# MarwanNour/SEAL-FYP-Logistic-Regression

Measured on AMD Instinct MI355X. Metric: CKKS ciphertext rotate+plain-mult ops/sec at N=16384; HBM GB/s vs roofline, higher is better.
Workload: dtype u64; 1 GPU; C3: N=16384, coeff_modulus bits [60, 40, 40, 40, 40, 60], level L=5 (k=6); per step and per GPU 4608 independent rotate_vector(step=1, direct Galois key)+multiply_plain, uniform random residues drawn on the device, inputs resident in HBM; batch_per_gpu=4608, parallelism=1 x independent ciphertext batches (no data-path collective), algorithmic_bytes_per_op=11141120

## Files before the change

### seal_fyp_logistic_regression_amd/csrc/hefx_keyswitch.hip

```cpp
#include <cstdio>
#include <cstdlib>
#include "hefx_internal.h"
#include "hefx_ntt.cuh"
#include "hefx_ntt8.cuh"

template <int LOGN>
struct KsWaves {
#ifdef HEFX_WAVES
    static constexpr int INV = HEFX_WAVES, FWD = HEFX_WAVES;
#else
    static constexpr int INV = LOGN <= 14 ? 2 : 4;
    static constexpr int FWD = LOGN <= 13 ? 2 : 4;
#endif
    static constexpr int NB_INV = (INV <= 2 && LOGN <= 13) ? 1 : 2, NB_FWD = (FWD <= 2 && LOGN < 13) ? 1 : 2;
};

namespace hefx {

typedef u64 u64x2_t __attribute__((ext_vector_type(2)));
__device__ __forceinline__ ulonglong2 nt_load16(const u64 *p)
{
    const u64x2_t v = __builtin_nontemporal_load(reinterpret_cast<const u64x2_t *>(p));
    return make_ulonglong2(v.x, v.y);
}
// ... 209 lines not shown
    struct Ctx {
        ModConst mc;
    };
    __device__ static __forceinline__ Ctx make(const ModConst &mc, const ModConstF &) { return Ctx{mc}; }
    typedef ulonglong2 X;
    struct K {
        ulonglong2 k0, k1;
    };
    __device__ static __forceinline__ X xin(const ulonglong2 &bits, bool, const Ctx &) { return bits; }
    __device__ static __forceinline__ K kin(const ulonglong2 &k0, const ulonglong2 &k1, const Ctx &) { return K{k0, k1}; }
    u64 a0xl = 0, a0xh = 0, a0yl = 0, a0yh = 0, a1xl = 0, a1xh = 0, a1yl = 0, a1yh = 0;
    __device__ __forceinline__ void mac(const X &x, const K &k, const Ctx &)
    {
        mac128(a0xl, a0xh, x.x, k.k0.x);
        mac128(a0yl, a0yh, x.y, k.k0.y);
        mac128(a1xl, a1xh, x.x, k.k1.x);
        mac128(a1yl, a1yh, x.y, k.k1.y);
    }
    __device__ __forceinline__ void mac_diag(const MacW &in, const ulonglong2 &dg, const Ctx &c)
    {
        ulonglong2 r0, r1;
        in.result(r0, r1, c);
        mac128(a0xl, a0xh, r0.x, dg.x);
        mac128(a0yl, a0yh, r0.y, dg.y);
        mac128(a1xl, a1xh, r1.x, dg.x);
        mac128(a1yl, a1yh, r1.y, dg.y);
    }
    template <bool LT2Q = false>
    __device__ __forceinline__ void result_data(ulonglong2 &r0, ulonglong2 &r1, const Ctx &c) const { result<LT2Q>(r0, r1, c); }
    template <bool LT2Q = false>
    __device__ __forceinline__ void result(ulonglong2 &r0, ulonglong2 &r1, const Ctx &c) const
    {
        r0.x = LT2Q ? barrett128_lt2q(a0xl, a0xh, c.mc) : barrett128(a0xl, a0xh, c.mc);
        r0.y = LT2Q ? barrett128_lt2q(a0yl, a0yh, c.mc) : barrett128(a0yl, a0yh, c.mc);
        r1.x = LT2Q ? barrett128_lt2q(a1xl, a1xh, c.mc) : barrett128(a1xl, a1xh, c.mc);
        r1.y = LT2Q ? barrett128_lt2q(a1yl, a1yh, c.mc) : barrett128(a1yl, a1yh, c.mc);
    }
};

struct MacL {
    typedef MacW::Ctx Ctx;
    __device__ static __forceinline__ Ctx make(const ModConst &mc, const ModConstF &) { return Ctx{mc}; }
    struct X {
        uint32_t xl, xh, yl, yh;
    };
    struct K {
        uint32_t k0xl, k0xh, k0yl, k0yh, k1xl, k1xh, k1yl, k1yh;
    };
    __device__ static __forceinline__ uint32_t lo30(u64 v) { return (uint32_t)v & 0x3FFFFFFFu; }
    __device__ static __forceinline__ uint32_t hi30(u64 v) { return (uint32_t)(v >> 30); }
    __device__ static __forceinline__ X xin(const ulonglong2 &b, bool, const Ctx &)
    {
        return X{lo30(b.x), hi30(b.x), lo30(b.y), hi30(b.y)};
    }
    __device__ static __forceinline__ K kin(const ulonglong2 &k0, const ulonglong2 &k1, const Ctx &)
    {
        return K{lo30(k0.x), hi30(k0.x), lo30(k0.y), hi30(k0.y), lo30(k1.x), hi30(k1.x), lo30(k1.y), hi30(k1.y)};
    }
    u64 c[4][3] = {};
    __device__ static __forceinline__ void mad(u64 (&col)[3], uint32_t xl, uint32_t xh, uint32_t kl, uint32_t kh)
    {
        col[0] += (u64)xl * kl;
        col[1] += (u64)xl * kh;
        col[1] += (u64)xh * kl;
        col[2] += (u64)xh * kh;
    }
    __device__ __forceinline__ void mac(const X &x, const K &k, const Ctx &)
    {
        mad(c[0], x.xl, x.xh, k.k0xl, k.k0xh);
        mad(c[1], x.yl, x.yh, k.k0yl, k.k0yh);
        mad(c[2], x.xl, x.xh, k.k1xl, k.k1xh);
        mad(c[3], x.yl, x.yh, k.k1yl, k.k1yh);
    }
    __device__ __forceinline__ void mac_diag(const MacL &in, const ulonglong2 &dg, const Ctx &cx)
    {
        ulonglong2 r0, r1;
        in.result(r0, r1, cx);
        const uint32_t dxl = lo30(dg.x), dxh = hi30(dg.x), dyl = lo30(dg.y), dyh = hi30(dg.y);
        mad(c[0], lo30(r0.x), hi30(r0.x), dxl, dxh);
        mad(c[1], lo30(r0.y), hi30(r0.y), dyl, dyh);
        mad(c[2], lo30(r1.x), hi30(r1.x), dxl, dxh);
        mad(c[3], lo30(r1.y), hi30(r1.y), dyl, dyh);
    }
    template <bool LT2Q>
    __device__ static __forceinline__ u64 fold(const u64 (&col)[3], const ModConst &mc)
    {
        u64 lo = col[0], hi = 0, t = col[1] << 30;
        lo += t;
        hi += (col[1] >> 34) + (lo < t);
        t = col[2] << 60;
        lo += t;
        hi += (col[2] >> 4) + (lo < t);
        return LT2Q ? barrett128_lt2q(lo, hi, mc) : barrett128(lo, hi, mc);
    }
    template <bool LT2Q = false>
    __device__ __forceinline__ void result_data(ulonglong2 &r0, ulonglong2 &r1, const Ctx &cx) const { result<LT2Q>(r0, r1, cx); }
    template <bool LT2Q = false>
    __device__ __forceinline__ void result(ulonglong2 &r0, ulonglong2 &r1, const Ctx &cx) const
    {
        r0.x = fold<LT2Q>(c[0], cx.mc);
        r0.y = fold<LT2Q>(c[1], cx.mc);
        r1.x = fold<LT2Q>(c[2], cx.mc);
        r1.y = fold<LT2Q>(c[3], cx.mc);
    }
};

struct MacF {
    typedef ArithF64::Ctx Ctx;
    __device__ static __forceinline__ Ctx make(const ModConst &, const ModConstF &mf) { return ArithF64::make(mf); }
    typedef double2 X;
    struct K {
        double k0x, k0y, k1x, k1y;
    };
    __device__ static __forceinline__ X xin(const ulonglong2 &b, bool own, const Ctx &)
    {
        return own ? make_double2(ArithF64::from_u64(b.x), ArithF64::from_u64(b.y))
                   : make_double2(__longlong_as_double((long long)b.x), __longlong_as_double((long long)b.y));
    }
    __device__ static __forceinline__ K kin(const ulonglong2 &k0, const ulonglong2 &k1, const Ctx &)
    {
        return K{ArithF64::from_u64(k0.x), ArithF64::from_u64(k0.y), ArithF64::from_u64(k1.x), ArithF64::from_u64(k1.y)};
    }
    double a0x = 0.0, a0y = 0.0, a1x = 0.0, a1y = 0.0;
    __device__ __forceinline__ void mac(const X &x, const K &k, const Ctx &c)
    {
        a0x += ArithF64::mm(x.x, k.k0x, c);
        a0y += ArithF64::mm(x.y, k.k0y, c);
        a1x += ArithF64::mm(x.x, k.k1x, c);
        a1y += ArithF64::mm(x.y, k.k1y, c);
    }
    __device__ __forceinline__ void mac_diag(const MacF &in, const ulonglong2 &dg, const Ctx &c)
    {
        const double dx = ArithF64::from_u64(dg.x), dy = ArithF64::from_u64(dg.y);
        a0x += ArithF64::mm(in.a0x, dx, c);
        a0y += ArithF64::mm(in.a0y, dy, c);
        a1x += ArithF64::mm(in.a1x, dx, c);
        a1y += ArithF64::mm(in.a1y, dy, c);
    }
    template <bool LT2Q = false>
    __device__ __forceinline__ void result_data(ulonglong2 &r0, ulonglong2 &r1, const Ctx &) const
    {
        r0.x = ArithF64::raw(a0x), r0.y = ArithF64::raw(a0y), r1.x = ArithF64::raw(a1x), r1.y = ArithF64::raw(a1y);
    }
    template <bool LT2Q = false>
    __device__ __forceinline__ void result(ulonglong2 &r0, ulonglong2 &r1, const Ctx &c) const
    {
        r0.x = ArithF64::canon(a0x, c);
        r0.y = ArithF64::canon(a0y, c);
        r1.x = ArithF64::canon(a1x, c);
        r1.y = ArithF64::canon(a1y, c);
    }
};

__device__ __forceinline__ bool slot_is_f64(const DevTables &T, int L, int jj)
{
    return T.modsf[jj < L ? jj : T.k - 1].q != 0.0;
}
__device__ __forceinline__ int nth_int_slot(const DevTables &T, int L, int y)
{
    int jj = 0;
    for (;; ++jj) {
        if (slot_is_f64(T, L, jj)) continue;
        if (y == 0) break;
        --y;
    }
    return jj;
}

template <class F>
__device__ __forceinline__ void mac_dispatch(const DevTables &T, int m, int L, const F &f)
{
    if (T.modsf[m].q != 0.0)
        f(MacF());
    else if (L <= 8 && (T.mods[m].q >> 60) == 0)
        f(MacL());
    else
        f(MacW());
}

template <bool STREAM>
__device__ __forceinline__ void mac_store(u64 *acc0, u64 *acc1, size_t w, const ulonglong2 &r0, const ulonglong2 &r1)
{
    if (STREAM) {
        nt_store16(acc0 + 2 * w, r0.x, r0.y);
        nt_store16(acc1 + 2 * w, r1.x, r1.y);
    } else {
        gst16(acc0 + 2 * w, r0);
        gst16(acc1 + 2 * w, r1);
    }
}

template <class P, int NI, bool STREAM, class XR>
__device__ __forceinline__ void mac_items(const DevTables &T, const u64 *key, int L, int jj, int m, size_t n, size_t w,
                                          const u64 *const (&own)[NI], const uint32_t (&own_elt)[NI], const XR &xrow,
                                          u64 *const (&acc0)[NI], u64 *const (&acc1)[NI])
{
    const typename P::Ctx cx = P::make(T.mods[m], T.modsf[m]);
    const int logn = T.logn;
    const size_t kpoly = (size_t)T.k * n;
    P A[NI];
    auto load_k = [&](int i, ulonglong2 &k0, ulonglong2 &k1) {
        const u64 *kb = key + ((size_t)i * 2 * T.k + m) * n;
        k0 = gld16(kb + 2 * w);
        k1 = gld16(kb + kpoly + 2 * w);
    };
    auto load_x = [&](int i, ulonglong2 (&xb)[NI]) {
#pragma unroll
        for (int e = 0; e < NI; ++e) {
            const u64 *xp = xrow(e, i) + 2 * w;
            xb[e] = STREAM ? nt_load16(xp) : gld16(xp);
        }
    };
    if (jj < L) {
        ulonglong2 xb[NI], k0, k1;
#pragma unroll
        for (int e = 0; e < NI; ++e) xb[e] = gather_pair(own[e], (uint32_t)w, own_elt[e], logn);
        load_k(jj, k0, k1);
        const typename P::K k = P::kin(k0, k1, cx);
#pragma unroll
        for (int e = 0; e < NI; ++e) A[e].mac(P::xin(xb[e], true, cx), k, cx);
    }
    constexpr int G = 1;
    auto digit_at = [&](int r) { return r < jj ? r : r + 1; };
    const int nd = jj < L ? L - 1 : L;
    int r0 = 0;
    for (; r0 + G <= nd; r0 += G) {
        ulonglong2 xb[G][NI], k0[G], k1[G];
#pragma unroll
        for (int g = 0; g < G; ++g) {
            load_x(digit_at(r0 + g), xb[g]);
            load_k(digit_at(r0 + g), k0[g], k1[g]);
        }
        HEFX_STAGE_FENCE();
#pragma unroll
        for (int g = 0; g < G; ++g) {
            const typename P::K k = P::kin(k0[g], k1[g], cx);
#pragma unroll
            for (int e = 0; e < NI; ++e) A[e].mac(P::xin(xb[g][e], false, cx), k, cx);
        }
    }
    for (; r0 < nd; ++r0) {
        ulonglong2 xb[NI], k0, k1;
        load_x(digit_at(r0), xb);
        load_k(digit_at(r0), k0, k1);
        const typename P::K k = P::kin(k0, k1, cx);
#pragma unroll
        for (int e = 0; e < NI; ++e) A[e].mac(P::xin(xb[e], false, cx), k, cx);
    }
#pragma unroll
    for (int e = 0; e < NI; ++e) {
        ulonglong2 r0, r1;
        if (jj < L) {
#ifdef HEFX_NO_LT2Q
            A[e].result_data(r0, r1, cx);
#else
            A[e].template result_data<true>(r0, r1, cx);
#endif
        } else {
#ifdef HEFX_NO_LT2Q
            A[e].result(r0, r1, cx);
#else
            A[e].template result<true>(r0, r1, cx);
#endif
        }
        mac_store<STREAM>(acc0[e], acc1[e], w, r0, r1);
    }
}

template <bool STREAM>
__device__ __forceinline__ void mac_unit(const DevTables &T, const KsItem *__restrict__ items, int L, int relin, int item0,
                                         int count, const KsScratch &S, int jj, int bl0, size_t w)
{
    const size_t n = (size_t)1 << T.logn;
    const int m = jj < L ? jj : T.k - 1;
    const bool two = bl0 + 1 < count;
    const KsItem it0 = items[item0 + bl0], it1 = items[item0 + bl0 + (two ? 1 : 0)];
    const int ownrow = jj < L ? jj : 0;
    const u64 *const own[2] = {it0.c_in + ((size_t)(relin ? 2 * L : L) + ownrow) * n,
                               it1.c_in + ((size_t)(relin ? 2 * L : L) + ownrow) * n};
    const uint32_t own_elt[2] = {relin ? 1u : item_elt(it0), relin ? 1u : item_elt(it1)};
    auto xrow2 = [&](int e, int i) { return S.x + (((size_t)(bl0 + e) * L + i) * (L + 1) + jj) * n; };
    auto accrow = [&](int bl, int c) { return S.acc + (((size_t)(item0 + bl) * 2 + c) * (L + 1) + jj) * n; };
    u64 *const acc0[2] = {accrow(bl0, 0), accrow(bl0 + 1, 0)}, *const acc1[2] = {accrow(bl0, 1), accrow(bl0 + 1, 1)};
    mac_dispatch(T, m, L, [&](auto pol) {
        using P = decltype(pol);
        if (two && it1.key == it0.key) {
            mac_items<P, 2, STREAM>(T, it0.key, L, jj, m, n, w, own, own_elt, xrow2, acc0, acc1);
        } else {
            const u64 *const o0[1] = {own[0]}, *const o1[1] = {own[1]};
            const uint32_t e0[1] = {own_elt[0]}, e1[1] = {own_elt[1]};
            u64 *const a00[1] = {acc0[0]}, *const a01[1] = {acc1[0]}, *const a10[1] = {acc0[1]}, *const a11[1] = {acc1[1]};
            mac_items<P, 1, STREAM>(T, it0.key, L, jj, m, n, w, o0, e0, [&](int, int i) { return xrow2(0, i); }, a00, a01);
            if (two)
                mac_items<P, 1, STREAM>(T, it1.key, L, jj, m, n, w, o1, e1, [&](int, int i) { return xrow2(1, i); }, a10, a11);
        }
    });
}

template <bool STREAM>
__global__ __launch_bounds__(256) void ks_mac_kernel(DevTables T, const KsItem *__restrict__ items, int L, int relin,
                                                     int item0, int count, int int_only, KsScratch S)
{
    if (S.gate_mode == 2 && ks_gated_out(S)) return;
    const int jj = int_only ? nth_int_slot(T, L, blockIdx.y) : (int)blockIdx.y;
#ifdef HEFX_STAMP
    const int wg = blockIdx.x + gridDim.x * (blockIdx.y + gridDim.y * blockIdx.z);
    if (threadIdx.x == 0 && wg < 1024) hefx_stamp_buf[((size_t)2 * 1024 + wg) * 16] = wall_clock64();
#endif
    mac_unit<STREAM>(T, items, L, relin, item0, count, S, jj, 2 * blockIdx.z, (size_t)blockIdx.x * blockDim.x + threadIdx.x);
#ifdef HEFX_STAMP
    if (HEFX_STAMP > 1) asm volatile("s_waitcnt vmcnt(0) lgkmcnt(0)" ::: "memory");
    if (threadIdx.x == 0 && wg < 1024) hefx_stamp_buf[((size_t)2 * 1024 + wg) * 16 + 15] = wall_clock64();
#endif
}

template <int LOGN>
__global__ __launch_bounds__(SplitCfg<LOGN>::T, KsWaves<LOGN>::FWD) void ks_ntt_digits_kernel(DevTables T, int L, int rows,
                                                                             int item0, int stream_x, KsScratch S)
{
    extern __shared__ __align__(16) u64 lds[];
    HEFX_STAMP_KERNEL(1);
    HEFX_STAMP_AT(0);
    ntt_digit_row<LOGN>(T, L, rows, item0, stream_x, S, lds);
    HEFX_STAMP_AT(15);
}

template <class P>
__device__ __forceinline__ void mac_gathered(P &A, const typename P::Ctx &cx, const DevTables &T, const KsItem &it,
                                             const u64 *__restrict__ c1, const KsScratch &S, int L, int jj, int m,
                                             size_t n, size_t w)
{
    const uint2 pi = gld_u32x2(it.perm + 2 * w);
    for (int i = 0; i < L; ++i) {
        const u64 *__restrict__ xrow = i == jj ? c1 + (size_t)i * n : S.x + ((size_t)i * (L + 1) + jj) * n;
        ulonglong2 xb;
        xb.x = gld8(xrow + pi.x);
        xb.y = gld8(xrow + pi.y);
        const u64 *kbase = it.key + ((size_t)i * 2 * T.k + m) * n;
        const ulonglong2 k0 = gld16(kbase + 2 * w);
        const ulonglong2 k1 = gld16(kbase + (size_t)T.k * n + 2 * w);
        A.mac(P::xin(xb, i == jj, cx), P::kin(k0, k1, cx), cx);
    }
}

__global__ __launch_bounds__(256) void ks_mac_exact_kernel(DevTables T, const KsItem *__restrict__ items, int L, KsScratch S)
{
    const size_t n = (size_t)1 << T.logn;
    const int jj = blockIdx.y, b = blockIdx.z;
    const int m = jj < L ? jj : T.k - 1;
    const size_t w = (size_t)blockIdx.x * blockDim.x + threadIdx.x;
    const KsItem it = items[b];
    if (w == 0 && jj == 0 && b == 0 && *S.gate == S.gate_tag) atomicAdd(S.gate_hits, 1u);
    const u64 *__restrict__ c1 = it.c_in + (size_t)L * n;
    const u64 *__restrict__ xs = S.x + (size_t)it.dsrc * L * (L + 1) * n;
    mac_dispatch(T, m, L, [&](auto pol) {
        using P = decltype(pol);
        const typename P::Ctx cx = P::make(T.mods[m], T.modsf[m]);
        P A, B;
        const uint32_t p0 = gld_u32x2(it.perm + 2 * w).x;
        const ulonglong2 wv = gld16(it.flipw + (size_t)m * n + 2 * w);
        auto load = [&](int i, const u64 *__restrict__ xrow, ulonglong2 &xb, ulonglong2 &k0, ulonglong2 &k1) {
            xb = gld16(xrow + (p0 & ~1u));
            const u64 *kbase = it.key + ((size_t)i * 2 * T.k + m) * n;
            k0 = gld16(kbase + 2 * w);
            k1 = gld16(kbase + (size_t)T.k * n + 2 * w);
        };
        auto swapped = [&](const ulonglong2 &v) { return (p0 & 1u) ? make_ulonglong2(v.y, v.x) : v; };
        if (jj < L) {
            ulonglong2 xb, k0, k1;
            load(jj, c1 + (size_t)jj * n, xb, k0, k1);
            A.mac(P::xin(swapped(xb), true, cx), P::kin(k0, k1, cx), cx);
        }
        constexpr int G = 1;
        auto digit_at = [&](int r) { return r < jj ? r : r + 1; };
        auto term = [&](int i, const ulonglong2 &xb, const ulonglong2 &k0, const ulonglong2 &k1) {
            const typename P::K k = P::kin(k0, k1, cx);
            A.mac(P::xin(swapped(xb), false, cx), k, cx);
            const u64 c = S.qmod[(size_t)i * T.k + m];
            B.mac(P::xin(make_ulonglong2(c, c), true, cx), k, cx);
        };
        const int nd = jj < L ? L - 1 : L;
        int r = 0;
        for (; r + G <= nd; r += G) {
            ulonglong2 xb[G], k0[G], k1[G];
#pragma unroll
            for (int g = 0; g < G; ++g) {
                const int i = digit_at(r + g);
                load(i, xs + ((size_t)i * (L + 1) + jj) * n, xb[g], k0[g], k1[g]);
            }
            HEFX_STAGE_FENCE();
#pragma unroll
            for (int g = 0; g < G; ++g) term(digit_at(r + g), xb[g], k0[g], k1[g]);
        }
        for (; r < nd; ++r) {
            const int i = digit_at(r);
            ulonglong2 xb, k0, k1;
            load(i, xs + ((size_t)i * (L + 1) + jj) * n, xb, k0, k1);
            term(i, xb, k0, k1);
        }
        ulonglong2 r0, r1, f0, f1;
        P C;
        C.mac_diag(B, wv, cx);
        if constexpr (std::is_same<P, MacF>::value) {
            if (jj < L) {
                P S2 = A;
                S2.a0x += C.a0x, S2.a0y += C.a0y, S2.a1x += C.a1x, S2.a1y += C.a1y;
                S2.result_data(r0, r1, cx);
            } else {
                A.result(r0, r1, cx);
                C.result(f0, f1, cx);
                const u64 q = T.mods[m].q;
                r0.x = addmod(r0.x, f0.x, q), r0.y = addmod(r0.y, f0.y, q);
                r1.x = addmod(r1.x, f1.x, q), r1.y = addmod(r1.y, f1.y, q);
            }
        } else {
            A.result(r0, r1, cx);
            C.result(f0, f1, cx);
            const u64 q = T.mods[m].q;
            r0.x = addmod(r0.x, f0.x, q);
            r0.y = addmod(r0.y, f0.y, q);
            r1.x = addmod(r1.x, f1.x, q);
            r1.y = addmod(r1.y, f1.y, q);
        }
        mac_store<false>(S.acc + (((size_t)b * 2 + 0) * (L + 1) + jj) * n, S.acc + (((size_t)b * 2 + 1) * (L + 1) + jj) * n,
                         w, r0, r1);
    });
}

__global__ __launch_bounds__(256) void flip_mask_kernel(DevTables T, const uint32_t *__restrict__ ginv, u64 *__restrict__ rows)
{
    const uint32_t n = 1u << T.logn;
    const uint32_t c = blockIdx.x * blockDim.x + threadIdx.x;
    const uint32_t e = blockIdx.z, m = blockIdx.y;
    rows[((size_t)e * T.k + m) * n + c] = ((c * ginv[e]) & (2 * n - 1)) >> T.logn;
}

constexpr int LT2_CHUNK = 8;

__global__ __launch_bounds__(256) void lt2_mac_kernel(DevTables T, const KsItem *__restrict__ items, int L, int nrot,
                                                      KsScratch S, const u64 *__restrict__ src_c1 ,
                                                      u64 *__restrict__ partial )
{
    const size_t n = (size_t)1 << T.logn;
    const int jj = blockIdx.y, ch = blockIdx.z;
    const int m = jj < L ? jj : T.k - 1;
    const size_t w = (size_t)blockIdx.x * blockDim.x + threadIdx.x;
    const int l0 = ch * LT2_CHUNK, l1 = l0 + LT2_CHUNK < nrot ? l0 + LT2_CHUNK : nrot;
    mac_dispatch(T, m, L, [&](auto pol) {
        using P = decltype(pol);
        const typename P::Ctx cx = P::make(T.mods[m], T.modsf[m]);
        P tot;
        for (int l = l0; l < l1; ++l) {
            const KsItem it = items[l];
            P A;
            mac_gathered(A, cx, T, it, src_c1, S, L, jj, m, n, w);
            tot.mac_diag(A, gld16(it.pt + (size_t)m * n + 2 * w), cx);
        }
        ulonglong2 r0, r1;
        tot.result(r0, r1, cx);
        u64 *base = partial + (size_t)ch * 2 * (L + 1) * n;
        mac_store<false>(base + (size_t)jj * n, base + ((size_t)(L + 1) + jj) * n, w, r0, r1);
    });
}

__global__ __launch_bounds__(256) void lt2_c0_kernel(DevTables T, const KsItem *__restrict__ items, int L, int nrot,
                                                     const u64 *__restrict__ c0, u64 *__restrict__ partial )
{
    const size_t n = (size_t)1 << T.logn;
    const int j = blockIdx.y, ch = blockIdx.z;
    const ModConst mc = T.mods[j];
    const size_t w = (size_t)blockIdx.x * blockDim.x + threadIdx.x;
    u64 xl = 0, xh = 0, yl = 0, yh = 0;
    const int l0 = ch * LT2_CHUNK, l1 = l0 + LT2_CHUNK < nrot ? l0 + LT2_CHUNK : nrot;
    const u64 *__restrict__ row = c0 + (size_t)j * n;
    for (int l = l0; l < l1; ++l) {
        const KsItem it = items[l];
        const uint2 pi = gld_u32x2(it.perm + 2 * w);
// ... 743 lines not shown
    int slot, g;
    fan_decode(4 * L, g, slot);
    const int j = slot >> 2, part = slot & 3;
    if (g >= rows) return;
    const int t = threadIdx.x;
    const int sp = T.k - 1;
    const ModConst mcp = T.mods[sp];
    const ModConstF mfp = T.modsf[sp];
    const NttTables ntp = ntt_tables(T, sp);
    const u64 *__restrict__ plane = S.u + (size_t)g * QC::N + (size_t)part * QC::Q;
    u64 v[8];
    if (mfp.q != 0.0)
        quarter_inv_planes<LOGN, ArithF64>(v, plane, lds, ntp.itwf, ArithF64::make(mfp), t);
    else
        quarter_inv_planes<LOGN, ArithU64>(v, plane, lds, ntp.itw, ArithU64::make(mcp), t);
    HEFX_STAMP_AT(15);
    HEFX_STAMP_KERNEL(4);
    HEFX_STAMP_AT(0);
    const u64 half = mcp.q >> 1;
#pragma unroll
    for (int r = 0; r < 8; ++r) v[r] = csub(v[r] + half, mcp.q);
    const ModConst mc = T.mods[j];
    const ModConstF mf = T.modsf[j];
    const InMode mode = {true, true, true, T.halfmod[(size_t)sp * T.k + j], true, mcp.q < 2 * mc.q};
    u64 *__restrict__ fd = S.x + ((size_t)g * L + j) * QC::N + (size_t)part * QC::Q;
    const NttTables nt = ntt_tables(T, j);
    fwd_policy_dispatch(mc, mf, [&](auto pol) {
        using A = decltype(pol);
        const typename A::Ctx cx = make_ctx(A{}, mc, mf);
        typename A::V f[8];
        fwd_inputs8<A>(f, v, mode, cx, mc);
        ntt8_fwd_core<LOGN - 2, A>(f, reinterpret_cast<typename A::V *>(lds), fwd_tw(A{}, nt), cx, t, 1);
#pragma unroll
        for (int r = 0; r < 8; r += 2) gst16(fd + C::idx_out(t, r), make_ulonglong2(A::raw(f[r]), A::raw(f[r + 1])));
    });
    HEFX_STAMP_AT(15);
}

template <int LOGN, class A>
__device__ __forceinline__ void pair_finish_body(const DevTables &T, const KsItem &it, int L, int relin, int b, int c, int j,
                                                 uint32_t g, const KsScratch &S)
{
    constexpr size_t N = (size_t)1 << LOGN, Q = N / 4;
    const int sp = T.k - 1;
    const ModConst mc = T.mods[j];
    const ModConstF mf = T.modsf[j];
    const typename A::Ctx cx = make_ctx(A{}, mc, mf);
    const auto pinv = md_pinv(A{}, T, sp, j);
    const typename A::TW *__restrict__ tw = fwd_tw(A{}, ntt_tables(T, j));
    const typename A::TW wb = tw[Q + g], wa0 = tw[2 * Q + 2 * g], wa1 = tw[2 * Q + 2 * g + 1];
    const u64 *__restrict__ fp = S.x + (((size_t)b * 2 + c) * L + j) * N + g;
    typename A::V p0 = A::unraw(gld8(fp)), p1 = A::unraw(gld8(fp + Q)), p2 = A::unraw(gld8(fp + 2 * Q)),
                  p3 = A::unraw(gld8(fp + 3 * Q));
    const size_t w4 = 4 * (size_t)g;
    const u64 *__restrict__ acc = S.acc + (((size_t)b * 2 + c) * (L + 1) + j) * N + w4;
    const ulonglong2 a01 = gld16(acc), a23 = gld16(acc + 2);
    const u64 *__restrict__ addrow = it.c_in + ((size_t)(relin ? c : 0) * L + j) * N;
    const bool has_add = relin || c == 0;
    const uint32_t elt = relin ? 1u : item_elt(it);
    const u64 *__restrict__ pt = it.pt ? it.pt + (size_t)j * N + w4 : nullptr;
    u64 *__restrict__ dst = it.c_out + ((size_t)c * L + j) * N + w4;
    auto epilogue = [&](auto has_add_c, auto has_pt_c) {
        constexpr bool HA = decltype(has_add_c)::value, HP = decltype(has_pt_c)::value;
        ulonglong2 s01 = make_ulonglong2(0, 0), s23 = s01, t01 = s01, t23 = s01;
        if constexpr (HA) {
            s01 = gather_pair(addrow, 2 * g, elt, LOGN);
            s23 = gather_pair(addrow, 2 * g + 1, elt, LOGN);
        }
        if constexpr (HP) {
            t01 = gld16(pt);
            t23 = gld16(pt + 2);
        }
        fwd_last_two<LOGN, A>(p0, p1, p2, p3, wb, wa0, wa1, cx);
        ulonglong2 o01, o23;
        o01.x = md_epilogue(A{}, p0, a01.x, s01.x, t01.x, HP, cx, pinv, mc);
        o01.y = md_epilogue(A{}, p1, a01.y, s01.y, t01.y, HP, cx, pinv, mc);
        o23.x = md_epilogue(A{}, p2, a23.x, s23.x, t23.x, HP, cx, pinv, mc);
        o23.y = md_epilogue(A{}, p3, a23.y, s23.y, t23.y, HP, cx, pinv, mc);
        gst16(dst, o01);
        gst16(dst + 2, o23);
        if constexpr (!HP) {
            if (it.acc_out) {
                const size_t arow = ((size_t)c * L + j) * N + w4;
                const ulonglong2 i01 = gld16(it.acc_in + arow), i23 = gld16(it.acc_in + arow + 2);
                gst16(it.acc_out + arow, make_ulonglong2(addmod(i01.x, o01.x, mc.q), addmod(i01.y, o01.y, mc.q)));
                gst16(it.acc_out + arow + 2, make_ulonglong2(addmod(i23.x, o23.x, mc.q), addmod(i23.y, o23.y, mc.q)));
            }
        }
    };
    if (has_add) {
        if (pt)
            epilogue(std::true_type{}, std::true_type{});
        else
            epilogue(std::true_type{}, std::false_type{});
    } else {
        if (pt)
            epilogue(std::false_type{}, std::true_type{});
        else
            epilogue(std::false_type{}, std::false_type{});
    }
}

template <int LOGN>
__global__ __launch_bounds__(256) void ks_pair_finish_kernel(DevTables T, const KsItem *__restrict__ items, int L, int relin,
                                                            KsScratch S)
{
    const int row = blockIdx.y, b = blockIdx.z;
    const int c = row / L, j = row % L;
    const uint32_t g = blockIdx.x * blockDim.x + threadIdx.x;
#ifdef HEFX_STAMP
    const int wg = blockIdx.x + gridDim.x * (blockIdx.y + gridDim.y * blockIdx.z);
    if (threadIdx.x == 0 && wg < 1024) hefx_stamp_buf[((size_t)5 * 1024 + wg) * 16] = wall_clock64();
#endif
    const KsItem it = items[b];
    const ModConst mc = T.mods[j];
    fwd_policy_dispatch(mc, T.modsf[j], [&](auto pol) {
        using A = decltype(pol);
        pair_finish_body<LOGN, A>(T, it, L, relin, b, c, j, g, S);
    });
#ifdef HEFX_STAMP
    if (HEFX_STAMP > 1) asm volatile("s_waitcnt vmcnt(0) lgkmcnt(0)" ::: "memory");
    if (threadIdx.x == 0 && wg < 1024) hefx_stamp_buf[((size_t)5 * 1024 + wg) * 16 + 15] = wall_clock64();
#endif
}

template <typename K>
static void set_lds(K kernel, size_t bytes)
{
    (void)hipFuncSetAttribute(reinterpret_cast<const void *>(kernel), hipFuncAttributeMaxDynamicSharedMemorySize,
                              (int)bytes);
}

template <int LOGN>
static hipError_t launch_keyswitch_chunk_t(const DevTables &T, int L, int n, const KsItem *batch, bool relin,
                                           const KsScratch &scr, int sub, bool alias,
                                           const KsSmallItems *small, int quarter, hipStream_t s, KsProf *prof, int nsrc)
{
    using SC = SplitCfg<LOGN>;
    const size_t lds = SC::LDS_BYTES;
    auto lds_knob = [lds](const char *name) {
        const char *e = getenv(name);
        const size_t v = e ? (size_t)atol(e) : 0;
        return v > lds ? v : lds;
    };
    static const size_t lds_fin = lds_knob("HEFX_FIN_LDS"), lds_ntt = lds_knob("HEFX_NTT_LDS"),
                        lds_intt = lds_knob("HEFX_INTT_LDS"), lds_mdi = lds_knob("HEFX_MDI_LDS");
    static PerDeviceOnce attr_once;
    if (attr_once.first()) {
        set_lds(ks_intt_digits_kernel<LOGN>, lds_intt);
        set_lds(ks_intt_digits_small_kernel<LOGN>, lds);
        set_lds(ks_ntt_digits_kernel<LOGN>, lds_ntt);
        set_lds(ks_moddown_intt_kernel<LOGN>, lds_mdi);
        set_lds(ks_moddown_finish_kernel<LOGN>, lds_fin);
        if (getenv("HEFX_DEBUG")) {
            int nb = -1;
            (void)hipOccupancyMaxActiveBlocksPerMultiprocessor(&nb, ks_ntt_digits_kernel<LOGN>, SC::T, lds);
            fprintf(stderr, "[hefx] ks_ntt_digits_kernel<%d>: %d threads, %zu B LDS -> %d workgroups/CU\n", LOGN, SC::T,
                    lds, nb);
        }
    }
    const int rl = relin ? 1 : 0;
    auto mark = [&](int stage) {
        if (prof && prof->used < prof->cap) {
            (void)hipEventRecord(prof->ev[prof->used], s);
            prof->stage[prof->used++] = stage;
        }
    };
    if (nsrc > 0) {
        KsScratch hs = scr, fb = scr;
        hs.gate_mode = 1;
        fb.gate_mode = 2;
        mark(1);
        hipLaunchKernelGGL((ks_intt_digits_kernel<LOGN>), dim3(split_grid(nsrc * L)), dim3(SC::T), lds_intt, s, T, batch + n, L,
                           0, 1, nsrc * L, hs);
        mark(2);
        hipLaunchKernelGGL((ks_ntt_digits_kernel<LOGN>), dim3(group_grid(nsrc * L, L)), dim3(SC::T), lds_ntt, s, T, L, nsrc * L,
                           0, 0, hs);
        mark(3);
        hipLaunchKernelGGL(ks_mac_exact_kernel, dim3(SC::N / 2 / 256, L + 1, n), dim3(256), 0, s, T, batch, L, hs);
        mark(4);
        hipLaunchKernelGGL((ks_moddown_intt_kernel<LOGN>), dim3(split_grid(n * 2)), dim3(SC::T), lds_mdi, s, T, L, n * 2, hs);
        mark(5);
        hipLaunchKernelGGL((ks_moddown_finish_kernel<LOGN>), dim3(group_grid(n * 2, L)), dim3(SC::T), lds_fin, s, T, batch, L,
                           0, n * 2, hs);
        mark(7);
        hipLaunchKernelGGL((ks_intt_digits_kernel<LOGN>), dim3(split_grid(n * L)), dim3(SC::T), lds_intt, s, T, batch, L, 0, 0,
                           n * L, fb);
        hipLaunchKernelGGL((ks_ntt_digits_kernel<LOGN>), dim3(group_grid(n * L, L)), dim3(SC::T), lds_ntt, s, T, L, n * L, 0, 0,
                           fb);
        hipLaunchKernelGGL(ks_mac_kernel<false>, dim3(SC::N / 2 / 256, L + 1, (n + 1) / 2), dim3(256), 0, s, T, batch, L, 0, 0, n,
                           0, fb);
        hipLaunchKernelGGL((ks_moddown_intt_kernel<LOGN>), dim3(split_grid(n * 2)), dim3(SC::T), lds_mdi, s, T, L, n * 2, fb);
        hipLaunchKernelGGL((ks_moddown_finish_kernel<LOGN>), dim3(group_grid(n * 2, L)), dim3(SC::T), lds_fin, s, T, batch, L,
                           0, n * 2, fb);
        mark(-1);
        return hipGetLastError();
    }
    if (small && (quarter & KS_Q_PAIR) && sub >= n) {
        static PerDeviceOnce attrp;
        const size_t ldsq = QuarterCfg<LOGN>::LDS_BYTES;
        if (attrp.first()) {
            set_lds(ks_pair_digits_kernel<LOGN>, ldsq);
            set_lds(ks_pair_moddown_kernel<LOGN>, ldsq);
        }
        constexpr int TQ = QuarterCfg<LOGN>::T;
        mark(1);
        hipLaunchKernelGGL((ks_pair_digits_kernel<LOGN>), fan_grid(n * L, 4 * L), dim3(TQ), ldsq, s, T, *small,
                           const_cast<KsItem *>(batch), n, L, rl, n * L, scr);
        mark(3);
        hipLaunchKernelGGL((ks_pair_mac_kernel<LOGN>), dim3(SC::N / 4 / 256, 2 * (L + 1), n), dim3(256), 0, s, T, batch, L, rl,
                           scr);
        mark(4);
        hipLaunchKernelGGL((ks_pair_moddown_kernel<LOGN>), fan_grid(n * 2, 4 * L), dim3(TQ), ldsq, s, T, L, n * 2,
                           scr);
        mark(5);
        hipLaunchKernelGGL((ks_pair_finish_kernel<LOGN>), dim3(SC::N / 4 / 256, 2 * L, n), dim3(256), 0, s, T, batch, L, rl,
                           scr);
        mark(-1);
        return hipGetLastError();
    }
    static const bool heavy_on = !(getenv("HEFX_HEAVY_FIRST") && atoi(getenv("HEFX_HEAVY_FIRST")) == 0);
    static const int heavy_max = getenv("HEFX_HEAVY_MAX") ? atoi(getenv("HEFX_HEAVY_MAX")) : 640;
    auto heavy_order = [&](int m) { return heavy_on && m * L * L * 2 <= heavy_max ? 2 : 0; };
    if (small && (quarter & KS_Q_ALL) && sub >= n) {
        static PerDeviceOnce attrq;
        const size_t ldsq = QuarterCfg<LOGN>::LDS_BYTES;
        if (attrq.first()) {
            set_lds(ks_intt_digits_q_kernel<LOGN>, ldsq);
            set_lds(ks_ntt_digits_q_kernel<LOGN>, ldsq);
            set_lds(ks_moddown_intt_q_kernel<LOGN>, ldsq);
            set_lds(ks_moddown_finish_q_kernel<LOGN>, ldsq);
        }
        constexpr int TQ = QuarterCfg<LOGN>::T;
        mark(1);
        if (quarter & KS_Q_INTT)
            hipLaunchKernelGGL((ks_intt_digits_q_kernel<LOGN>), dim3(quarter_grid(n * L)), dim3(TQ), ldsq, s, T, *small,
                               const_cast<KsItem *>(batch), n, L, rl, n * L, scr);
        else
            hipLaunchKernelGGL((ks_intt_digits_small_kernel<LOGN>), dim3(split_grid(n * L)), dim3(SC::T), lds, s, T, *small,
                               const_cast<KsItem *>(batch), n, L, rl, n * L, scr);
        mark(2);
        if (quarter & KS_Q_NTT)
            hipLaunchKernelGGL((ks_ntt_digits_q_kernel<LOGN>), fan_grid(n * L, 4 * L), dim3(TQ), ldsq, s, T, L,
                               n * L, scr);
        else
            hipLaunchKernelGGL((ks_ntt_digits_kernel<LOGN>), dim3(group_grid(n * L, L)), dim3(SC::T), lds_ntt, s, T, L,
                               n * L, 0, heavy_order(n), scr);
        mark(3);
        hipLaunchKernelGGL(ks_mac_kernel<false>, dim3(SC::N / 2 / 256, L + 1, (n + 1) / 2), dim3(256), 0, s, T, batch, L, rl, 0,
                           n, 0, scr);
        mark(4);
        if (quarter & KS_Q_MDI)
            hipLaunchKernelGGL((ks_moddown_intt_q_kernel<LOGN>), dim3(quarter_grid(n * 2)), dim3(TQ), ldsq, s, T, L, n * 2,
                               scr);
        else
            hipLaunchKernelGGL((ks_moddown_intt_kernel<LOGN>), dim3(split_grid(n * 2)), dim3(SC::T), lds_mdi, s, T, L, n * 2,
                               scr);
        mark(5);
        if (quarter & KS_Q_FIN)
            hipLaunchKernelGGL((ks_moddown_finish_q_kernel<LOGN>), fan_grid(n * 2, 4 * L), dim3(TQ), ldsq, s, T,
                               batch, L, rl, n * 2, scr);
        else
            hipLaunchKernelGGL((ks_moddown_finish_kernel<LOGN>), dim3(group_grid(n * 2, L)), dim3(SC::T), lds_fin, s, T,
                               batch, L, rl, n * 2, scr);
        mark(-1);
        return hipGetLastError();
    }
    static const int force_stream_x = getenv("HEFX_STREAM_X") ? atoi(getenv("HEFX_STREAM_X")) : -1;
    auto stream_x_of = [&](int m) {
        return force_stream_x >= 0 ? force_stream_x : ((size_t)m * L * (L + 1) * SC::N * 8 > ((size_t)256 << 20) ? 1 : 0);
    };
    if (alias) {
        mark(0);
        hipLaunchKernelGGL(ks_alias_copy_kernel, dim3(SC::N / 2 / 256, 2 * L, n), dim3(256), 0, s, T, batch, L);
    }
    mark(1);
    if (small)
        hipLaunchKernelGGL((ks_intt_digits_small_kernel<LOGN>), dim3(split_grid(n * L)), dim3(SC::T), lds, s, T, *small,
                           const_cast<KsItem *>(batch), n, L, rl, n * L, scr);
    else
        hipLaunchKernelGGL((ks_intt_digits_kernel<LOGN>), dim3(split_grid(n * L)), dim3(SC::T), lds_intt, s, T, batch, L, rl, 0,
                           n * L, scr);
    if (sub < 0) {
        if constexpr (LOGN <= 14) {
            static PerDeviceOnce fattr;
            if (fattr.first()) set_lds(ks_ntt_macf_kernel<LOGN>, FusedCfg<LOGN>::LDS_BYTES);
            const int code = -sub - 1, nf = code & 0xff;
            const bool special_int = (code >> 8) & 1;
            const int nint = L + 1 - nf;
            const int pairs = special_int ? (nint - 1) * (L - 1) + L : nint * (L - 1);
            const int per_item = 2 * (nf + pairs);
            const int stream_x = (size_t)n * pairs * SC::N * 8 > ((size_t)256 << 20) ? 1 : 0;
            mark(6);
            hipLaunchKernelGGL((ks_ntt_macf_kernel<LOGN>), dim3(((n + 7) / 8) * 8 * per_item), dim3(FusedCfg<LOGN>::T),
                               FusedCfg<LOGN>::LDS_BYTES, s, T, batch, L, rl, n, nf, per_item, stream_x, scr);
            if (nint > 0) {
                mark(3);
                if (stream_x)
                    hipLaunchKernelGGL(ks_mac_kernel<true>, dim3(SC::N / 2 / 256, nint, (n + 1) / 2), dim3(256), 0, s, T, batch,
                                       L, rl, 0, n, 1, scr);
                else
                    hipLaunchKernelGGL(ks_mac_kernel<false>, dim3(SC::N / 2 / 256, nint, (n + 1) / 2), dim3(256), 0, s, T, batch,
                                       L, rl, 0, n, 1, scr);
            }
        }
    } else
    for (int item0 = 0; item0 < n; item0 += sub) {
        const int m = n - item0 < sub ? n - item0 : sub;
        mark(2);
        const int stream_x = stream_x_of(m);
        hipLaunchKernelGGL((ks_ntt_digits_kernel<LOGN>), dim3(group_grid(m * L, L)), dim3(SC::T), lds_ntt, s, T, L, m * L,
                           item0, stream_x | heavy_order(m), scr);
        mark(3);
        if (stream_x)
            hipLaunchKernelGGL(ks_mac_kernel<true>, dim3(SC::N / 2 / 256, L + 1, (m + 1) / 2), dim3(256), 0, s, T, batch,
                               L, rl, item0, m, 0, scr);
        else
            hipLaunchKernelGGL(ks_mac_kernel<false>, dim3(SC::N / 2 / 256, L + 1, (m + 1) / 2), dim3(256), 0, s, T, batch,
                               L, rl, item0, m, 0, scr);
    }
    mark(4);
    hipLaunchKernelGGL((ks_moddown_intt_kernel<LOGN>), dim3(split_grid(n * 2)), dim3(SC::T), lds_mdi, s, T, L, n * 2, scr);
    mark(5);
    hipLaunchKernelGGL((ks_moddown_finish_kernel<LOGN>), dim3(group_grid(n * 2, L)), dim3(SC::T), lds_fin, s, T, batch, L,
                       rl, n * 2, scr);
    mark(-1);
    return hipGetLastError();
}

__global__ __launch_bounds__(256) void lt2_reduce_kernel(DevTables T, int L, int period, int rows, int chunks,
                                                         const u64 *__restrict__ partial, const u64 *addin, u64 *out)
{
    const size_t n = (size_t)1 << T.logn;
    const int r = blockIdx.y;
    const int jj = r % period;
    const u64 q = T.mods[jj < L ? jj : T.k - 1].q;
    const size_t w = (size_t)blockIdx.x * blockDim.x + threadIdx.x;
    ulonglong2 acc = addin ? reinterpret_cast<const ulonglong2 *>(addin + (size_t)r * n)[w] : make_ulonglong2(0, 0);
    for (int ch = 0; ch < chunks; ++ch) {
        const ulonglong2 v = reinterpret_cast<const ulonglong2 *>(partial + ((size_t)ch * rows + r) * n)[w];
        acc.x = addmod(acc.x, v.x, q);
        acc.y = addmod(acc.y, v.y, q);
    }
    if (period == L + 1 && jj < L && T.modsf[jj].q != 0.0)
        acc = make_ulonglong2(ArithF64::raw(ArithF64::from_u64(acc.x)), ArithF64::raw(ArithF64::from_u64(acc.y)));
    reinterpret_cast<ulonglong2 *>(out + (size_t)r * n)[w] = acc;
}

template <int LOGN>
static hipError_t launch_lt2_decompose_t(const DevTables &T, int L, const KsItem *src_item, const KsItem *rot_items,
                                         int nrot, const KsScratch &scr, const u64 *ct_new, u64 *partial_s,
                                         u64 *partial_c0, u64 *cbuf, hipStream_t s)
{
    using SC = SplitCfg<LOGN>;
    const size_t lds = SC::LDS_BYTES;
    static PerDeviceOnce attr_once;
    if (attr_once.first()) {
        set_lds(ks_intt_digits_kernel<LOGN>, lds);
        set_lds(ks_ntt_digits_kernel<LOGN>, lds);
        set_lds(ks_moddown_intt_kernel<LOGN>, lds);
        set_lds(ks_moddown_finish_kernel<LOGN>, lds);
    }
    const int chunks = (nrot + LT2_CHUNK - 1) / LT2_CHUNK;
    hipLaunchKernelGGL((ks_intt_digits_kernel<LOGN>), dim3(split_grid(L)), dim3(SC::T), lds, s, T, src_item, L, 0, 1, L,
                       scr);
    hipLaunchKernelGGL((ks_ntt_digits_kernel<LOGN>), dim3(group_grid(L, L)), dim3(SC::T), lds, s, T, L, L, 0, 0, scr);
    hipLaunchKernelGGL(lt2_mac_kernel, dim3(SC::N / 2 / 256, L + 1, chunks), dim3(256), 0, s, T, rot_items, L, nrot, scr,
                       ct_new + (size_t)L * SC::N, partial_s);
    hipLaunchKernelGGL(lt2_c0_kernel, dim3(SC::N / 2 / 256, L, chunks), dim3(256), 0, s, T, rot_items, L, nrot, ct_new,
                       partial_c0);
    hipLaunchKernelGGL(lt2_reduce_kernel, dim3(SC::N / 2 / 256, 2 * (L + 1)), dim3(256), 0, s, T, L, L + 1, 2 * (L + 1),
                       chunks, partial_s, (const u64 *)nullptr, scr.acc);
    hipLaunchKernelGGL(lt2_reduce_kernel, dim3(SC::N / 2 / 256, L), dim3(256), 0, s, T, L, L, L, chunks, partial_c0,
                       (const u64 *)cbuf, cbuf);
    return hipGetLastError();
}
template <int LOGN>
static hipError_t launch_lt2_moddown_t(const DevTables &T, int L, const KsItem *item, const KsScratch &scr, hipStream_t s)
{
    using SC = SplitCfg<LOGN>;
    const size_t lds = SC::LDS_BYTES;
    hipLaunchKernelGGL((ks_moddown_intt_kernel<LOGN>), dim3(split_grid(2)), dim3(SC::T), lds, s, T, L, 2, scr);
    hipLaunchKernelGGL((ks_moddown_finish_kernel<LOGN>), dim3(group_grid(2, L)), dim3(SC::T), lds, s, T, item, L, 1, 2,
                       scr);
    return hipGetLastError();
}

#ifdef HEFX_ONLY_LOGN
#define HEFX_DISPATCH_SPLIT(logn, CALL) \
    if ((logn) == HEFX_ONLY_LOGN) return CALL(HEFX_ONLY_LOGN); \
    return hipErrorInvalidValue;
#else
#define HEFX_DISPATCH_SPLIT(logn, CALL)       \
    switch (logn) {                           \
        case 11: return CALL(11);             \
        case 12: return CALL(12);             \
        case 13: return CALL(13);             \
        case 14: return CALL(14);             \
        case 15: return CALL(15);             \
        default: return hipErrorInvalidValue; \
    }
#endif

hipError_t launch_lt2_decompose(const DevTables &T, int L, const KsItem *src_item, const KsItem *rot_items, int nrot,
                                const KsScratch &scr, const u64 *ct_new, u64 *partial_s, u64 *partial_c0, u64 *cbuf,
                                hipStream_t s)
{
#define CALL(LN) launch_lt2_decompose_t<LN>(T, L, src_item, rot_items, nrot, scr, ct_new, partial_s, partial_c0, cbuf, s)
    HEFX_DISPATCH_SPLIT(T.logn, CALL)
#undef CALL
}
hipError_t launch_lt2_moddown(const DevTables &T, int L, const KsItem *item, const KsScratch &scr, hipStream_t s)
{
#define CALL(LN) launch_lt2_moddown_t<LN>(T, L, item, scr, s)
    HEFX_DISPATCH_SPLIT(T.logn, CALL)
#undef CALL
}
int lt2_chunk() { return LT2_CHUNK; }

int ks_small_max() { return KS_SMALL_MAX; }
hipError_t launch_keyswitch_chunk(const DevTables &T, int L, int n, const KsItem *batch, bool relin,
                                  const KsScratch &scr, int sub, bool alias, const KsItem *small_items,
                                  int quarter, hipStream_t s, KsProf *prof, int nsrc)
{
    KsSmallItems sm;
    const KsSmallItems *small = nullptr;
    if (small_items && n <= KS_SMALL_MAX && !nsrc && !alias) {
        for (int i = 0; i < n; ++i) sm.it[i] = small_items[i];
        for (int i = n; i < KS_SMALL_MAX; ++i) sm.it[i] = KsItem{};
        small = &sm;
    }
    if (T.logn < 12) quarter = 0;
#define CALL(LN) launch_keyswitch_chunk_t<LN>(T, L, n, batch, relin, scr, sub, alias, small, quarter, s, prof, nsrc)
    HEFX_DISPATCH_SPLIT(T.logn, CALL)
#undef CALL
}

hipError_t launch_flip_rows(const DevTables &T, const uint32_t *d_ginv, int count, u64 *rows, hipStream_t s)
{
    hipLaunchKernelGGL(flip_mask_kernel, dim3((1u << T.logn) / 256, T.k, count), dim3(256), 0, s, T, d_ginv, rows);
    return hipGetLastError();
}

template <int LOGN>
__global__ __launch_bounds__(SplitCfg<LOGN>::T, KsWaves<LOGN>::INV) void rs_intt_kernel(DevTables T, int L, int size, int rows,
                                                                       const u64 *in, const u64 *const *__restrict__ tab,
                                                                       u64 *d, int rounded)
{
    using SC = SplitCfg<LOGN>;
    using C = typename SC::C;
    extern __shared__ __align__(16) u64 lds[];
    int p, h;
    split_decode(blockIdx.x, p, h);
    if (p >= rows) return;
    const int t = threadIdx.x;
    const u64 *__restrict__ base = tab ? tab[p / size] + (size_t)(p % size) * L * SC::N : in + (size_t)p * L * SC::N;
    const ulonglong2 *__restrict__ src = reinterpret_cast<const ulonglong2 *>(base + (size_t)(L - 1) * SC::N);
    u64 v[16];
    split_inv<LOGN, KsWaves<LOGN>::NB_INV>(v, src, lds, ntt_tables(T, L - 1), T.mods[L - 1], T.modsf[L - 1], t, h);
    u64 *__restrict__ dd = d + (size_t)p * SC::N + (size_t)h * SC::H;
    const u64 ql = T.mods[L - 1].q, half = rounded ? ql >> 1 : 0;
#pragma unroll
    for (int r = 0; r < 16; ++r) dd[C::idx_nat(t, r)] = csub(v[r] + half, ql);
// ... 155 lines not shown
```

Before: 242,500 rotate+multiply_plain ops/s.

## Fuse digit INTT with half-size forward NTT modup and finish last butterfly in MAC

```diff
diff --git a/seal_fyp_logistic_regression_amd/csrc/hefx_keyswitch.hip b/seal_fyp_logistic_regression_amd/csrc/hefx_keyswitch.hip
--- a/seal_fyp_logistic_regression_amd/csrc/hefx_keyswitch.hip
+++ b/seal_fyp_logistic_regression_amd/csrc/hefx_keyswitch.hip
@@ -385,6 +385,21 @@
     }
 };
 
+__device__ __forceinline__ double modup_zeta(MacF, const NttTables &nt, size_t k) { return nt.twf[k]; }
+template <class P>
+__device__ __forceinline__ ulonglong2 modup_zeta(P, const NttTables &nt, size_t k) { return nt.tw[k]; }
+__device__ __forceinline__ ulonglong2 modup_last(MacF, const ulonglong2 &eo, double z, const ArithF64::Ctx &c)
+{
+    const double e = ArithF64::unraw(eo.x), t = ArithF64::mm(ArithF64::unraw(eo.y), z, c);
+    return make_ulonglong2(ArithF64::raw(e + t), ArithF64::raw(e - t));
+}
+template <class P>
+__device__ __forceinline__ ulonglong2 modup_last(P, const ulonglong2 &eo, const ulonglong2 &z, const MacW::Ctx &c)
+{
+    const u64 t = csubn(shoup_lazy(eo.y, z.x, z.y, c.mc.nq), c.mc.nq);
+    return make_ulonglong2(csubn(eo.x + t, c.mc.nq), csubn(eo.x + c.mc.q - t, c.mc.nq));
+}
+
 __device__ __forceinline__ bool slot_is_f64(const DevTables &T, int L, int jj)
 {
     return T.modsf[jj < L ? jj : T.k - 1].q != 0.0;
@@ -423,7 +438,7 @@
     }
 }
 
-template <class P, int NI, bool STREAM, class XR>
+template <class P, int NI, bool STREAM, bool MODUP, class XR>
 __device__ __forceinline__ void mac_items(const DevTables &T, const u64 *key, int L, int jj, int m, size_t n, size_t w,
                                           const u64 *const (&own)[NI], const uint32_t (&own_elt)[NI], const XR &xrow,
                                           u64 *const (&acc0)[NI], u64 *const (&acc1)[NI])
@@ -437,12 +452,31 @@
         k0 = gld16(kb + 2 * w);
         k1 = gld16(kb + kpoly + 2 * w);
     };
+    const size_t hn = n / 2;
+    const auto zeta = [&] {
+        if constexpr (MODUP)
+            return modup_zeta(P{}, ntt_tables(T, m), hn + w);
+        else
+            return 0;
+    }();
     auto load_x = [&](int i, ulonglong2 (&xb)[NI]) {
 #pragma unroll
         for (int e = 0; e < NI; ++e) {
-            const u64 *xp = xrow(e, i) + 2 * w;
-            xb[e] = STREAM ? nt_load16(xp) : gld16(xp);
-        }
+            if constexpr (MODUP) {
+                const u64 *xp = xrow(e, i) + w;
+                xb[e] = STREAM ? make_ulonglong2(__builtin_nontemporal_load(xp), __builtin_nontemporal_load(xp + hn))
+                               : make_ulonglong2(gld8(xp), gld8(xp + hn));
+            } else {
+                const u64 *xp = xrow(e, i) + 2 * w;
+                xb[e] = STREAM ? nt_load16(xp) : gld16(xp);
+            }
+        }
+    };
+    auto xop = [&](const ulonglong2 &xb) {
+        if constexpr (MODUP)
+            return P::xin(modup_last(P{}, xb, zeta, cx), false, cx);
+        else
+            return P::xin(xb, false, cx);
     };
     if (jj < L) {
         ulonglong2 xb[NI], k0, k1;
@@ -469,7 +503,7 @@
         for (int g = 0; g < G; ++g) {
             const typename P::K k = P::kin(k0[g], k1[g], cx);
 #pragma unroll
-            for (int e = 0; e < NI; ++e) A[e].mac(P::xin(xb[g][e], false, cx), k, cx);
+            for (int e = 0; e < NI; ++e) A[e].mac(xop(xb[g][e]), k, cx);
         }
     }
     for (; r0 < nd; ++r0) {
@@ -478,7 +512,7 @@
         load_k(digit_at(r0), k0, k1);
         const typename P::K k = P::kin(k0, k1, cx);
 #pragma unroll
-        for (int e = 0; e < NI; ++e) A[e].mac(P::xin(xb[e], false, cx), k, cx);
+        for (int e = 0; e < NI; ++e) A[e].mac(xop(xb[e]), k, cx);
     }
 #pragma unroll
     for (int e = 0; e < NI; ++e) {
@@ -500,7 +534,7 @@
     }
 }
 
-template <bool STREAM>
+template <bool STREAM, bool MODUP>
 __device__ __forceinline__ void mac_unit(const DevTables &T, const KsItem *__restrict__ items, int L, int relin, int item0,
                                          int count, const KsScratch &S, int jj, int bl0, size_t w)
 {
@@ -518,19 +552,19 @@
     mac_dispatch(T, m, L, [&](auto pol) {
         using P = decltype(pol);
         if (two && it1.key == it0.key) {
-            mac_items<P, 2, STREAM>(T, it0.key, L, jj, m, n, w, own, own_elt, xrow2, acc0, acc1);
+            mac_items<P, 2, STREAM, MODUP>(T, it0.key, L, jj, m, n, w, own, own_elt, xrow2, acc0, acc1);
         } else {
             const u64 *const o0[1] = {own[0]}, *const o1[1] = {own[1]};
             const uint32_t e0[1] = {own_elt[0]}, e1[1] = {own_elt[1]};
             u64 *const a00[1] = {acc0[0]}, *const a01[1] = {acc1[0]}, *const a10[1] = {acc0[1]}, *const a11[1] = {acc1[1]};
-            mac_items<P, 1, STREAM>(T, it0.key, L, jj, m, n, w, o0, e0, [&](int, int i) { return xrow2(0, i); }, a00, a01);
+            mac_items<P, 1, STREAM, MODUP>(T, it0.key, L, jj, m, n, w, o0, e0, [&](int, int i) { return xrow2(0, i); }, a00, a01);
             if (two)
-                mac_items<P, 1, STREAM>(T, it1.key, L, jj, m, n, w, o1, e1, [&](int, int i) { return xrow2(1, i); }, a10, a11);
+                mac_items<P, 1, STREAM, MODUP>(T, it1.key, L, jj, m, n, w, o1, e1, [&](int, int i) { return xrow2(1, i); }, a10, a11);
         }
     });
 }
 
-template <bool STREAM>
+template <bool STREAM, bool MODUP = false>
 __global__ __launch_bounds__(256) void ks_mac_kernel(DevTables T, const KsItem *__restrict__ items, int L, int relin,
                                                      int item0, int count, int int_only, KsScratch S)
 {
@@ -540,7 +574,7 @@
     const int wg = blockIdx.x + gridDim.x * (blockIdx.y + gridDim.y * blockIdx.z);
     if (threadIdx.x == 0 && wg < 1024) hefx_stamp_buf[((size_t)2 * 1024 + wg) * 16] = wall_clock64();
 #endif
-    mac_unit<STREAM>(T, items, L, relin, item0, count, S, jj, 2 * blockIdx.z, (size_t)blockIdx.x * blockDim.x + threadIdx.x);
+    mac_unit<STREAM, MODUP>(T, items, L, relin, item0, count, S, jj, 2 * blockIdx.z, (size_t)blockIdx.x * blockDim.x + threadIdx.x);
 #ifdef HEFX_STAMP
     if (HEFX_STAMP > 1) asm volatile("s_waitcnt vmcnt(0) lgkmcnt(0)" ::: "memory");
     if (threadIdx.x == 0 && wg < 1024) hefx_stamp_buf[((size_t)2 * 1024 + wg) * 16 + 15] = wall_clock64();
@@ -556,6 +590,65 @@
     HEFX_STAMP_AT(0);
     ntt_digit_row<LOGN>(T, L, rows, item0, stream_x, S, lds);
     HEFX_STAMP_AT(15);
+}
+
+template <int LOGN, class A>
+__device__ __forceinline__ void modup_target(const DevTables &T, const u64 *__restrict__ dd, const InMode &mode, int m,
+                                             u64 *__restrict__ xd, int stream_x, u64 *lds, int t)
+{
+    using C = NttCfg<LOGN - 1>;
+    static_assert(C::R != 0, "idx_out is the store layout (idx_io) only for R > 0");
+    const ModConst mc = T.mods[m];
+    const typename A::Ctx cx = make_ctx(A{}, mc, T.modsf[m]);
+    typename A::V f[16];
+    if (A::IS_F64 ? mode.red_f64 : mode.red_int) {
+#pragma unroll
+        for (int r = 0; r < 16; ++r) f[r] = A::template input<1>(dd[C::idx_nat(t, r)], mode, cx, mc);
+    } else {
+#pragma unroll
+        for (int r = 0; r < 16; ++r) f[r] = A::template input<0>(dd[C::idx_nat(t, r)], mode, cx, mc);
+    }
+    __syncthreads();
+    ntt_fwd_core<LOGN - 1, A, NoHook, true>(f, reinterpret_cast<typename A::V *>(lds), fwd_tw(A{}, ntt_tables(T, m)), cx, t, 1);
+    u64 v[16];
+#pragma unroll
+    for (int r = 0; r < 16; ++r) v[r] = A::mac_operand(f[r], cx);
+    if (stream_x & 1) {
+#pragma unroll
+        for (int r = 0; r < 16; r += 2) nt_store16(xd + C::idx_out(t, r), v[r], v[r + 1]);
+    } else {
+#pragma unroll
+        for (int r = 0; r < 16; r += 2)
+            *reinterpret_cast<ulonglong2 *>(xd + C::idx_out(t, r)) = make_ulonglong2(v[r], v[r + 1]);
+    }
+}
+
+template <int LOGN>
+__global__ __launch_bounds__(SplitCfg<LOGN>::T, KsWaves<LOGN>::FWD) void ks_modup_kernel(DevTables T, const KsItem *__restrict__ items,
+                                                                        int L, int relin, int rows, int item0,
+                                                                        int stream_x, KsScratch S)
+{
+    using SC = SplitCfg<LOGN>;
+    extern __shared__ __align__(16) u64 lds[];
+    int p, h;
+    split_decode(blockIdx.x, p, h);
+    if (p >= rows) return;
+    const int t = threadIdx.x;
+    const int bl = p / L, i = p % L, b = item0 + bl;
+    intt_digits_body<LOGN>(T, items[b], L, relin, 0, b, i, h, S, lds);
+    const u64 *__restrict__ dd = S.d + ((size_t)b * L + i) * SC::N + (size_t)h * SC::H;
+    const u64 qi = T.mods[i].q;
+    const bool wide_i = T.modsf[i].q == 0.0;
+    for (int r = 0; r < L; ++r) {
+        int tl = t;
+        asm volatile("" : "+v"(tl));
+        const int jj = r >= i ? r + 1 : r;
+        const int m = jj < L ? jj : T.k - 1;
+        const InMode mode = {qi > T.mods[m].q, wide_i, false, 0};
+        u64 *__restrict__ xd = S.x + (((size_t)bl * L + i) * (L + 1) + jj) * SC::N + (size_t)h * SC::H;
+        fwd_policy_dispatch(T.mods[m], T.modsf[m],
+                            [&](auto pol) { modup_target<LOGN, decltype(pol)>(T, dd, mode, m, xd, stream_x, lds, tl); });
+    }
 }
 
 template <class P>
@@ -1605,6 +1698,7 @@
         set_lds(ks_ntt_digits_kernel<LOGN>, lds_ntt);
         set_lds(ks_moddown_intt_kernel<LOGN>, lds_mdi);
         set_lds(ks_moddown_finish_kernel<LOGN>, lds_fin);
+        if constexpr (LOGN == 14) set_lds(ks_modup_kernel<LOGN>, lds);
         if (getenv("HEFX_DEBUG")) {
             int nb = -1;
             (void)hipOccupancyMaxActiveBlocksPerMultiprocessor(&nb, ks_ntt_digits_kernel<LOGN>, SC::T, lds);
@@ -1727,11 +1821,13 @@
         mark(0);
         hipLaunchKernelGGL(ks_alias_copy_kernel, dim3(SC::N / 2 / 256, 2 * L, n), dim3(256), 0, s, T, batch, L);
     }
+    static const bool modup_on = !(getenv("HEFX_MODUP") && atoi(getenv("HEFX_MODUP")) == 0);
+    const bool modup = LOGN == 14 && modup_on && !small && sub > 0;
     mark(1);
     if (small)
         hipLaunchKernelGGL((ks_intt_digits_small_kernel<LOGN>), dim3(split_grid(n * L)), dim3(SC::T), lds, s, T, *small,
                            const_cast<KsItem *>(batch), n, L, rl, n * L, scr);
-    else
+    else if (!modup)
         hipLaunchKernelGGL((ks_intt_digits_kernel<LOGN>), dim3(split_grid(n * L)), dim3(SC::T), lds_intt, s, T, batch, L, rl, 0,
                            n * L, scr);
     if (sub < 0) {
@@ -1762,6 +1858,20 @@
         const int m = n - item0 < sub ? n - item0 : sub;
         mark(2);
         const int stream_x = stream_x_of(m);
+        if (modup) {
+            if constexpr (LOGN == 14) {
+                hipLaunchKernelGGL((ks_modup_kernel<LOGN>), dim3(split_grid(m * L)), dim3(SC::T), lds, s, T, batch, L, rl, m * L,
+                                   item0, stream_x, scr);
+                mark(3);
+                if (stream_x)
+                    hipLaunchKernelGGL((ks_mac_kernel<true, true>), dim3(SC::N / 2 / 256, L + 1, (m + 1) / 2), dim3(256), 0, s, T,
+                                       batch, L, rl, item0, m, 0, scr);
+                else
+                    hipLaunchKernelGGL((ks_mac_kernel<false, true>), dim3(SC::N / 2 / 256, L + 1, (m + 1) / 2), dim3(256), 0, s, T,
+                                       batch, L, rl, item0, m, 0, scr);
+            }
+            continue;
+        }
         hipLaunchKernelGGL((ks_ntt_digits_kernel<LOGN>), dim3(group_grid(m * L, L)), dim3(SC::T), lds_ntt, s, T, L, m * L,
                            item0, stream_x | heavy_order(m), scr);
         mark(3);
```

Result: faster. 244,900 rotate+multiply_plain ops/s, median of 6 (+1.0%).
